# SEEDtk/kmers.anno

Hardware: AMD Instinct MI355X
Metric: kmer lookups/s + seqs annotated/s at 1/2/4/8 GPUs; achieved HBM GB/s vs roofline (higher is better)
Workload: dtype u64; 1 GPU; c5: 1M proteins per rank vs 10^8-entry multi-function signature table (HBM random access); proteins_per_gpu=1000000, windows_per_gpu=303576763, batch_windows=303576763, table_entries=100000000, functions=100000, k=8, min_hits=5, table_layout_m=6, table_minimizer_order=mod-sampling, table_placement=two-choice, parallelism=input-shard x1, table on this GPU

## Files before the change

kmers.anno_amd/csrc/kma_internal.h:

```cpp
#pragma once

#include <hip/hip_runtime.h>
#include <stdint.h>

#include "../../include/kmeranno.h"

namespace kma {

#ifndef KMA_BUCKET_SLOTS
#define KMA_BUCKET_SLOTS 8
#endif
constexpr int kSlotsPerBucket = KMA_BUCKET_SLOTS;
static_assert(kSlotsPerBucket == 8 || kSlotsPerBucket == 16, "64- or 128-byte buckets");
constexpr int kBucketBytes = kSlotsPerBucket * 8;
constexpr int kBucketHalves = kBucketBytes / 64;
constexpr int kSlotBits = kSlotsPerBucket == 16 ? 4 : 3;
#ifndef KMA_FILTER_BITS
#define KMA_FILTER_BITS 2
#endif
constexpr int kFilterBits = KMA_FILTER_BITS;
static_assert(kFilterBits >= 1 && kFilterBits <= 3, "one to three filter bits per slot");
constexpr uint32_t kFidBits = 24 - kFilterBits;
constexpr uint32_t kFidMask = (1u << kFidBits) - 1;
constexpr uint32_t kKeyHiMask = 0xFF000000u;
// ... 50 lines not shown
}
__host__ __device__ inline uint32_t mix32_lite(uint32_t h) {
  h ^= h >> 16;
  h *= 0x7FEB352Du;
  h ^= h >> 15;
  return h;
}
__host__ __device__ inline uint32_t parity32(uint32_t x) {
#ifdef __HIP_DEVICE_COMPILE__
  return (uint32_t)__popc(x) & 1u;
#else
  return (uint32_t)__builtin_popcount(x) & 1u;
#endif
}

__host__ __device__ inline uint32_t mmer_hash(uint32_t sub) {
#if KMA_HASH_LITE
  return sub * 0x9E3779B1u;
#else
  return mix32(sub * 0x9E3779B1u + 0x7F4A7C15u);
#endif
}
constexpr int kOrderMod = KMA_LAYOUT_MOD_SAMPLING;
constexpr int kMinimizerMask = 0x3F;
__host__ __device__ constexpr bool order_mod_valid(int k, int m) {
  return k == 8 && (m & kMinimizerMask) == 6;
}
__host__ __device__ inline uint32_t mod_sample(uint64_t key) {
  uint32_t best = 0xFFFFFFFFu;
  for (int i = 0; i < 8; ++i) {
    const uint32_t c = (uint32_t)(key >> (5 * (7 - i))) & 31u;
    const uint32_t g = (31u - c) << 5 | (uint32_t)(4 * i);
    best = best < g ? best : g;
  }
  const uint32_t lo = (uint32_t)key, hi = (uint32_t)(key >> 32);
#ifdef __HIP_DEVICE_COMPILE__
  const uint32_t sh = __builtin_amdgcn_ubfe(0x5A05A05Au, best, 4u);
  const uint32_t sub = __builtin_amdgcn_alignbit(hi, lo, sh) & 0x3FFFFFFFu;
#else
  const uint32_t sh = (0x5A05A05Au >> (best & 31u)) & 15u;
  const uint32_t sub = (uint32_t)(((uint64_t)hi << 32 | lo) >> sh) & 0x3FFFFFFFu;
#endif
  return mmer_hash(sub);
}
__host__ __device__ inline uint32_t minimizer_hash(uint64_t key, int k, int m) {
  if (m & kOrderMod) return mod_sample(key);
  const uint32_t mask = (uint32_t)((1ull << (5 * m)) - 1);
  uint32_t best = 0xFFFFFFFFu;
  for (int p = 0; p <= k - m; ++p) {
    const uint32_t h = mmer_hash((uint32_t)(key >> (5 * (k - m - p))) & mask);
    best = best < h ? best : h;
  }
  return best;
}

__host__ __device__ inline uint32_t home_from_hash(uint32_t h, uint64_t key, int m,
                                                   uint32_t n_buckets) {
  if (m != 0 && n_buckets >= 2) {
    const uint32_t pair = (uint32_t)(((uint64_t)h * (n_buckets >> 1)) >> 32);
#if KMA_HASH_LITE
    return 2u * pair + parity32((uint32_t)key);
#else
    return 2u * pair + (((uint32_t)key * 0x2C1B3C6Du) >> 31);
#endif
  }
  return (uint32_t)(((uint64_t)h * n_buckets) >> 32);
}
__host__ __device__ inline uint32_t home_from_min(uint32_t mn, uint64_t key, int m,
                                                  uint32_t n_buckets) {
#if KMA_HASH_LITE
  return home_from_hash(mix32_lite(mn ^ 0x85EBCA77u), key, m, n_buckets);
#else
  return home_from_hash(mix32(mn ^ 0x85EBCA77u), key, m, n_buckets);
#endif
}
__host__ __device__ inline uint32_t home_bucket(uint64_t key, int k, int m, uint32_t n_buckets) {
  if (m == 0)
    return home_from_hash(mix32((uint32_t)key ^ mix32((uint32_t)(key >> 32) + 0x9E3779B9u)),
                          key, m, n_buckets);
  return home_from_min(minimizer_hash(key, k, m), key, m, n_buckets);
}

#ifndef KMA_CHAIN_HASH
#define KMA_CHAIN_HASH 1
#endif
constexpr uint32_t kHashChainMin = 1024;
constexpr uint32_t kChainStepSearch = 4096;
__host__ __device__ inline bool chain_hashed(uint32_t n_buckets) {
  return KMA_CHAIN_HASH && n_buckets >= kHashChainMin;
}
__host__ __device__ inline uint32_t chain_bucket(uint32_t home, uint32_t i, uint32_t n_buckets) {
  if (chain_hashed(n_buckets)) {
    if (i == 0u) return home;
    const uint32_t r = (uint32_t)(((uint64_t)mix32(home * 0x9E3779B1u ^ i * 0x85EBCA77u) *
                                   (n_buckets - 1u)) >> 32);
    const uint32_t b = home + 1u + r;
    return b >= n_buckets ? b - n_buckets : b;
  }
  const uint64_t b = (uint64_t)home + i;
  return (uint32_t)(b >= n_buckets ? b - n_buckets : b);
}
__host__ __device__ inline uint32_t chain_step(uint32_t home, uint32_t b, uint32_t n_buckets) {
  if (chain_hashed(n_buckets)) {
    for (uint32_t i = 0; i < kChainStepSearch; ++i)
      if (chain_bucket(home, i, n_buckets) == b) return i;
    return kChainStepSearch;
  }
  return b >= home ? b - home : b + n_buckets - home;
}

__host__ __device__ inline uint32_t alt_bucket(uint64_t key, uint32_t home, uint32_t n_buckets) {
  const uint32_t h = mix32((uint32_t)key * 0x2C1B3C6Du ^ mix32_lite((uint32_t)(key >> 32) + 0x68E31DA5u));
  const uint32_t b = (uint32_t)(((uint64_t)h * (n_buckets - 1u)) >> 32);
  return b >= home ? b + 1u : b;
}
constexpr uint32_t kMaxKicks = 2000;
constexpr int kLayoutTwoChoice = KMA_LAYOUT_TWO_CHOICE;
constexpr int kLayoutMask = 0xFF;
constexpr double kMaxDisplacedTwoChoice = 0.40;

constexpr uint64_t kMinimizer6Buckets = kSlotsPerBucket == 16 ? (1ull << 24) : (1ull << 25);
constexpr uint64_t kMinimizer6BucketsWide = 1ull << 26;
int minimizer_len(int k, uint64_t n_buckets);
constexpr double kRetryDisplaced = 0.10;
constexpr double kMaxDisplaced = 0.15;
constexpr uint32_t kMaxChain = 32;

#ifndef KMA_BLOCK_PROTEINS
#define KMA_BLOCK_PROTEINS 8
#endif
#ifndef KMA_SET_POOL
#define KMA_SET_POOL 4096
#endif
#ifndef KMA_PROBE_WIN
#define KMA_PROBE_WIN (KMA_BUCKET_SLOTS == 16 ? 1 : 2)
#endif
constexpr int kProbeWin = KMA_PROBE_WIN;
constexpr int kBlockProteins = KMA_BLOCK_PROTEINS;
constexpr int kSetPool = KMA_SET_POOL;
#ifndef KMA_LANE_PERM
#define KMA_LANE_PERM 1
#endif
#ifndef KMA_CHAIN_Q
#define KMA_CHAIN_Q 192
#endif
constexpr int kChainQ = KMA_CHAIN_Q;
static_assert(kChainQ >= 64 * (kProbeWin + 1), "chain queue below two steps of windows");
constexpr uint32_t kGlobalSet = 0xFFFFFFFFu;
constexpr int kWavesPerBlock = 4;
#ifndef KMA_PROTEIN_OCC
#define KMA_PROTEIN_OCC 7
#endif
constexpr int kProteinOcc = KMA_PROTEIN_OCC;
#ifndef KMA_STAGE_RES
#define KMA_STAGE_RES 1024
#endif
constexpr int kStageRes = KMA_STAGE_RES;
constexpr int kStageGroups = kStageRes / 8 + 1;
constexpr int kStageEntries = (5 * kStageGroups + 15) / 16 * 4;
static_assert(kStageRes % (256 * kProbeWin) == 0, "a stage holds whole probe steps");
static_assert(4 * kStageEntries >= 5 * kStageRes / 8 + 8, "the last window reads two aligned words");
static_assert(kStageEntries < kSetPool / 2, "the stage leaves most of the pool to the sets");

struct ProteinArgs {
  const uint64_t* slots;
  uint32_t n_buckets;
  const uint8_t* lut;
  const uint8_t* residues;
  const uint64_t* offsets;
  uint32_t n_seq;
  uint32_t n_residues;
  int32_t k;
  int32_t mlen;
  int32_t min_hits;
  uint32_t flags;
  int32_t* out_fid;
  int32_t* out_count;
  uint8_t* out_status;
  uint32_t* tally;
  uint32_t n_fid;
  uint32_t* gset;
  uint32_t block_proteins;
  uint32_t defer_below;
  uint32_t n_groups;
  uint32_t packed;
  uint64_t stream_first;
  uint32_t two_choice;
};

struct ContigArgs {
  const uint64_t* slots;
  uint32_t n_buckets;
  const uint8_t* dna;
  const uint64_t* offsets;
  uint32_t n_contig;
  uint64_t total_bases;
  int32_t k;
  int32_t mlen;
  kma_hit* staging;
  uint32_t* block_counts;
  uint64_t* group_sum;
  uint32_t* emit_done;
  uint32_t n_groups;
  uint32_t groups_scanned;
  uint32_t* tally;
  uint32_t n_fid;
  kma_hit* out;
  uint64_t cap;
  uint64_t* n_hits;
  uint32_t* slot_count;
  int32_t strict_pass;
  uint32_t two_choice;
  uint8_t codon_codes[64];
};
#ifndef KMA_CONTIG_POS
#define KMA_CONTIG_POS 1
#endif
constexpr int kContigPos = KMA_CONTIG_POS;
#ifndef KMA_CONTIG_SEQ
#define KMA_CONTIG_SEQ 4
#endif
constexpr int kContigSeq = KMA_CONTIG_SEQ;
static_assert(kContigSeq == 1 || kContigPos == 1, "sequential slices take one position per lane");
constexpr int kContigTile = 256 * kContigPos * kContigSeq;
constexpr uint32_t kScanGroup = 256;
constexpr uint32_t kDirectGroups = 1024;

struct PropArgs {
  const kma_hit* hits;
  uint32_t n;
  const uint32_t* peg_len;
  uint32_t n_peg;
  int32_t k;
  double min_strength, max_fuzz, min_fuzz;
  uint32_t *keys, *skeys, *idx, *sidx;
  uint32_t *head, *list_no, *starts;
  uint32_t* scontig;
  int32_t* sleft;
  uint32_t *keep, *evidence, *out_pos;
  int32_t* best;
  uint64_t* stats;
  kma_proposal* out;
  uint64_t cap;
};
hipError_t launch_propose(PropArgs a, void* temp, size_t* temp_bytes, hipStream_t stream);

hipError_t launch_build_insert(uint64_t* slots, uint32_t* winner, uint32_t n_buckets, int k,
                               int m, const uint64_t* keys, uint64_t n, uint32_t* status,
                               hipStream_t stream);
hipError_t launch_build_finalize(uint64_t* slots, const uint32_t* winner, const uint32_t* fids,
                                 uint32_t n_buckets, int k, int m, uint32_t* stats,
                                 hipStream_t stream);
struct TwoChoiceScratch {
  uint32_t* home = nullptr;
  uint32_t* sorted_home = nullptr;
  uint32_t* sorted_idx = nullptr;
  uint8_t* away = nullptr;
  uint8_t* load = nullptr;
};
hipError_t launch_build_two_choice(uint64_t* slots, uint32_t n_buckets, int k, int m,
                                   const uint64_t* keys, const uint32_t* fids, uint64_t n,
                                   uint64_t* sorted_keys, uint32_t* rows, uint32_t* sorted_rows,
                                   const TwoChoiceScratch& x, void* temp, size_t* temp_bytes,
                                   uint32_t* status, hipStream_t stream);
hipError_t launch_annotate(const ProteinArgs& a, hipStream_t stream);
hipError_t launch_pack_residues(const uint8_t* residues, const uint64_t* offsets, uint64_t n,
                                const uint8_t* lut, uint8_t* out, hipStream_t stream);
__host__ __device__ constexpr uint64_t packed_bytes(uint64_t n) { return 40 * ((n + 63) / 64) + 16; }
hipError_t launch_contigs_emit(const ContigArgs& a, uint64_t n_blocks, hipStream_t stream);
hipError_t launch_contigs_probe(const ContigArgs& a, uint64_t n_blocks, hipStream_t stream);
hipError_t launch_peg_windows(const uint8_t* residues, const uint64_t* offsets, uint32_t n_peg,
                              int k, const uint8_t* lut, uint64_t* keys, uint32_t* pegs,
                              hipStream_t stream);
hipError_t launch_sort_pairs(void* temp, size_t* temp_bytes, const uint64_t* keys_in,
                             uint64_t* keys_out, const uint32_t* vals_in, uint32_t* vals_out,
                             uint64_t n, int key_bits, hipStream_t stream);
hipError_t launch_singleton_flags(const uint64_t* sorted_keys, uint64_t n, uint8_t* flags,
                                  hipStream_t stream);
constexpr uint32_t kBuildNeg = 0xFFFFFFu;
hipError_t launch_build_windows(const uint8_t* residues, const uint64_t* offsets, uint32_t n_seq,
                                const int32_t* roles, int k, int end_exclusive, const uint8_t* lut,
                                uint64_t* keys, uint32_t* tags, uint32_t* alpha_flag,
                                hipStream_t stream);
hipError_t launch_signature_flags(const uint64_t* keys, const uint32_t* tags, uint64_t n,
                                  uint8_t* flags, uint32_t* head_idx, uint32_t* run, void* temp,
                                  size_t* temp_bytes, hipStream_t stream);
hipError_t launch_select_flagged(void* temp, size_t* temp_bytes, const uint64_t* keys_in,
                                 const uint32_t* vals_in, const uint8_t* flags, uint64_t* keys_out,
                                 uint32_t* vals_out, uint64_t* n_out, uint64_t n,
                                 hipStream_t stream);

}
```

kmers.anno_amd/csrc/kma_kernels.hip:

```cpp
#include <cstring>
#include <rocprim/rocprim.hpp>

#include <algorithm>
#include <cstdio>
#include <cstdlib>

#include "../../include/kmeranno.h"
#include "kma_internal.h"
#include "kma_device.h"


namespace kma {
namespace {


template <bool Wide>
__global__ __launch_bounds__(256) void build_insert_kernel(uint64_t* slots, uint32_t* winner,
                                                           uint32_t n_buckets, int k, int m,
                                                           const uint64_t* __restrict__ keys,
                                                           uint64_t n, uint32_t* status) {
  constexpr int S = Wide ? kWideSlots : kSlotsPerBucket;
  for (uint64_t i = blockIdx.x * (uint64_t)blockDim.x + threadIdx.x; i < n;
       i += (uint64_t)gridDim.x * blockDim.x) {
    const uint64_t key = keys[i];
// ... 183 lines not shown
    while (e < n && hs[e] == h && e - i < 64) ++e;
    const uint32_t W = (uint32_t)(e - i);
    for (uint64_t j = i; j < e; ++j) away[ids[j]] = 0;
    if (W <= S) continue;
    uint64_t chosen = 0;
    uint32_t set = 0;
    for (uint32_t it = 0; it < W - S; ++it) {
      uint32_t best = 0, best_new = 64, best_mask = 0;
      for (uint32_t j = 0; j < W; ++j) {
        if (chosen >> j & 1ull) continue;
        const uint64_t key = skeys[ids[i + j]];
        const uint32_t mask = filter_need<S>((uint32_t)key);
        const bool alt_full = load && load[alt_bucket(key, h, n_buckets)] >= S;
        const uint32_t fresh = (uint32_t)__popc(mask & ~set) + (alt_full ? 32u : 0u);
        if (fresh < best_new) {
          best = j;
          best_new = fresh;
          best_mask = mask;
          if (fresh == 0) break;
        }
      }
      chosen |= 1ull << best;
      set |= best_mask;
      away[ids[i + best]] = 1;
    }
  }
}

__global__ __launch_bounds__(256) void build_two_choice_filter_kernel(uint64_t* slots,
                                                                      uint32_t n_buckets, int k,
                                                                      int m, uint32_t* stats) {
  constexpr int S = kSlotsPerBucket;
  const uint64_t n_slots = (uint64_t)n_buckets * S;
  uint32_t entries = 0, displaced = 0;
  for (uint64_t i = blockIdx.x * (uint64_t)blockDim.x + threadIdx.x; i < n_slots;
       i += (uint64_t)gridDim.x * blockDim.x) {
    const uint64_t v = __hip_atomic_load(slots + i, __ATOMIC_RELAXED, __HIP_MEMORY_SCOPE_AGENT);
    if ((uint32_t)v == 0u) continue;
    const uint64_t key = slot_key(v);
    const uint32_t b = (uint32_t)(i / S), h = home_bucket(key, k, m, n_buckets);
    entries++;
    if (b != h) {
      displaced++;
      for (int f = 0; f < kFilterBits; ++f) {
        const uint32_t pos = filter_pos<S>((uint32_t)key, f);
        uint32_t* meta = reinterpret_cast<uint32_t*>(slots + (uint64_t)h * S + pos / kFilterBits) + 1;
        const uint32_t bit = 1u << (kFidBits + pos % kFilterBits);
        if (!(__hip_atomic_load(meta, __ATOMIC_RELAXED, __HIP_MEMORY_SCOPE_AGENT) & bit))
          atomicOr(meta, bit);
      }
    }
  }
  entries = wave_sum(entries);
  displaced = wave_sum(displaced);
  if ((threadIdx.x & 63) == 0) {
    if (entries) atomicAdd(stats + 0, entries);
    atomicMax(stats + 1, displaced ? 2u : entries ? 1u : 0u);
    if (displaced) atomicAdd(stats + 2, displaced);
  }
}


#ifdef KMA_BLOCK_CLOCK
__device__ uint64_t g_block_clk[8 * 65536];
#define KMA_CLK_SET(i, v)                                          \
  do {                                                             \
    if (threadIdx.x == 0 && blockIdx.x < 65535)                    \
      g_block_clk[8 * blockIdx.x + (i)] = (v);                     \
  } while (0)
#define KMA_CLK(i) KMA_CLK_SET(i, wall_clock64())
#define KMA_CLK_HW()                                                \
  KMA_CLK_SET(6, (uint64_t)__builtin_amdgcn_s_getreg(20 | (15 << 11)) << 32 | \
                     (uint32_t)__builtin_amdgcn_s_getreg(4 | (31 << 11)))
#else
#define KMA_CLK_SET(i, v) ((void)0)
#define KMA_CLK(i) ((void)0)
#define KMA_CLK_HW() ((void)0)
#endif

#ifdef KMA_TUNE_COUNT
__device__ unsigned long long g_walk_stats[8];
#define KMA_COUNT(i, v)                                                                    \
  do {                                                                                     \
    const unsigned long long kma_v_ = (unsigned long long)(v);   \
    if ((threadIdx.x & 63) == 0)                                                           \
      __hip_atomic_fetch_add(&g_walk_stats[i], kma_v_, __ATOMIC_RELAXED,                   \
                             __HIP_MEMORY_SCOPE_AGENT);                                    \
  } while (0)
#else
#define KMA_COUNT(i, v) ((void)0)
#endif

template <int P>
struct ProteinSmem {
  __attribute__((aligned(16))) uint32_t pool[kSetPool];
  uint32_t chain_q[kWavesPerBlock][2 * kChainQ];
  uint32_t pbeg[P + 1];
  uint32_t pwin[P];
  uint32_t pset[P];
  uint32_t pcap[P];
  uint32_t pmin[P], pmax[P], pcnt[P];
  uint32_t plist[P];
  uint32_t skip;
  uint8_t lut[256];
};
static_assert(sizeof(ProteinSmem<kBlockProteins>) <= 163840 / kProteinOcc,
              "protein-path LDS must leave kProteinOcc blocks per CU");

__device__ __forceinline__ bool lds_set_insert(uint32_t* set, uint32_t cap, uint32_t key) {
  uint32_t i = set_slot(key, cap);
  for (;;) {
    const uint32_t o = atomicCAS(set + i, 0u, key);
    if (o == 0u) return true;
    if (o == key) return false;
    i = i + 1 == cap ? 0u : i + 1;
  }
}
__device__ __forceinline__ bool global_set_insert(uint32_t* set, uint32_t cap, uint32_t key) {
  uint32_t i = set_slot(key, cap);
  for (;;) {
    uint32_t o = 0u;
    __hip_atomic_compare_exchange_strong(set + i, &o, key, __ATOMIC_RELAXED, __ATOMIC_RELAXED,
                                         __HIP_MEMORY_SCOPE_AGENT);
    if (o == 0u) return true;
    if (o == key) return false;
    i = i + 1 == cap ? 0u : i + 1;
  }
}

template <int P>
__device__ __forceinline__ void record_hit(ProteinSmem<P>& sm, const ProteinArgs& a,
                                           uint64_t span_lo, bool multiset, uint32_t p,
                                           uint32_t fid, uint32_t sid) {
  atomicMin(&sm.pmin[p], fid);
  atomicMax(&sm.pmax[p], fid);
  bool fresh = true;
#ifdef KMA_TUNE_NO_SET
  fresh = false;
  if (false) {
#else
  if (!multiset) {
#endif
    const uint32_t base = sm.pset[p];
    if (base != kGlobalSet) {
      fresh = lds_set_insert(sm.pool + base, sm.pcap[p], sid + 1u);
    } else {
      a.gset[2 * (span_lo + sm.pbeg[p]) + atomicAdd(&sm.plist[p], 1u)] = sid + 1u;
      fresh = false;
    }
  }
  if (fresh) atomicAdd(&sm.pcnt[p], 1u);
}

template <int P>
__device__ __forceinline__ void dedupe_lists(ProteinSmem<P>& sm, const ProteinArgs& a,
                                             uint64_t span_lo) {
  const int t = threadIdx.x;
  for (int p = 0; p < P; ++p) {
    if (sm.pset[p] != kGlobalSet) continue;
    if (sm.pmin[p] != sm.pmax[p]) continue;
    const uint32_t h = sm.plist[p], b0 = sm.pbeg[p];
    if (h == 0) continue;
    const uint32_t* list = a.gset + 2 * (span_lo + b0);
    uint32_t fresh = 0;
    if (h < (uint32_t)kSetPool) {
      uint4* pool4 = reinterpret_cast<uint4*>(sm.pool);
      for (uint32_t i = t; i < (uint32_t)kSetPool / 4; i += 256) pool4[i] = make_uint4(0u, 0u, 0u, 0u);
      __syncthreads();
      for (uint32_t i = t; i < h; i += 256) fresh += lds_set_insert(sm.pool, kSetPool, list[i]);
    } else {
      const uint32_t L = sm.pbeg[p + 1] - b0;
      uint32_t* set = a.gset + 2 * (span_lo + b0) + L;
      for (uint32_t i = t; i < L; i += 256)
        __hip_atomic_store(set + i, 0u, __ATOMIC_RELAXED, __HIP_MEMORY_SCOPE_AGENT);
      __threadfence();
      __syncthreads();
      for (uint32_t i = t; i < h; i += 256) fresh += global_set_insert(set, L, list[i]);
    }
    fresh = wave_sum(fresh);
    if ((t & 63) == 0 && fresh) atomicAdd(&sm.pcnt[p], fresh);
    __syncthreads();
  }
}

template <int P>
__device__ __forceinline__ uint32_t dead_mask(const ProteinSmem<P>& sm) {
  uint32_t lane;
  asm volatile("v_mbcnt_lo_u32_b32 %0, -1, 0\n\tv_mbcnt_hi_u32_b32 %0, -1, %0" : "=v"(lane));
  const uint32_t i = lane < (uint32_t)P ? lane : 0u;
  const uint32_t mn = sm.pmin[i], mx = sm.pmax[i];
  return (uint32_t)__ballot(lane < (uint32_t)P && mx > mn);
}

template <int P>
__device__ __forceinline__ uint32_t protein_at(const uint32_t (&pb)[P + 1], uint32_t x) {
  uint32_t p = 0;
#pragma unroll
  for (int i = 1; i < P; ++i) p += x >= pb[i] ? 1u : 0u;
  return p;
}
template <int P>
__device__ __forceinline__ bool window_at(const uint32_t (&pe)[P], uint32_t x, uint32_t p) {
  uint32_t ended = 0;
#pragma unroll
  for (int i = 0; i < P; ++i) ended += x >= pe[i] ? 1u : 0u;
  return ended == p;
}

__device__ __forceinline__ uint32_t lane_window(int t) {
#if KMA_LANE_PERM
  return (uint32_t)((t >> 6) * 64 + 16 * (t & 3) + ((t & 63) >> 2));
#else
  return (uint32_t)t;
#endif
}

#ifndef KMA_XCD_GROUPS
#define KMA_XCD_GROUPS 1
#endif
__device__ __forceinline__ uint32_t xcd_group(uint32_t b, uint32_t n) {
#if KMA_XCD_GROUPS
  const uint32_t per = n >> 3;
  return b < 8u * per ? (b & 7u) * per + (b >> 3) : b;
#else
  (void)n;
  return b;
#endif
}

struct GroupHead {
  uint32_t p0, np;
  uint64_t beg_raw;
  uint64_t span_lo;
};
__device__ __forceinline__ void head_offsets(const ProteinArgs& a, uint32_t g, GroupHead& h) {
  const int lane = threadIdx.x & 63, wave = threadIdx.x >> 6;
  h.p0 = g * a.block_proteins;
  h.np = min(a.block_proteins, a.n_seq - h.p0);
  h.beg_raw = wave == 0 && lane <= (int)h.np ? a.offsets[h.p0 + lane] : 0u;
  h.span_lo = a.offsets[h.p0] - a.offsets[0];
}
template <bool Packed>
__device__ __forceinline__ const uint8_t* head_res(const ProteinArgs& a, const GroupHead& h,
                                                   uint64_t& pos0) {
  if (Packed) {
    pos0 = a.stream_first + h.span_lo;
    return a.residues;
  }
  const uint8_t* res0 = a.residues + a.offsets[0] + h.span_lo;
  pos0 = (uintptr_t)res0 & 7u;
  return res0 - pos0;
}
template <int U>
__device__ __forceinline__ void head_residues(const ProteinArgs& a, const GroupHead& h,
                                              uint32_t tw, WinWords (&ww)[U]) {
  uint64_t pos0;
  const uint8_t* res = head_res<true>(a, h, pos0);
  const uint64_t lim = a.n_residues - h.span_lo;
#pragma unroll
  for (int j = 0; j < U; ++j) {
    const uint32_t x = j * 256u + tw;
    ww[j] = window_words_packed(res, (x < lim ? x : 0u) + pos0);
  }
}

constexpr int kStagePerThread = (kStageGroups + 255) / 256;
static_assert(kStagePerThread <= kProbeWin, "a lane's stage words wait in its window registers");
__device__ __forceinline__ void stage_fetch(const uint8_t* __restrict__ res, uint32_t xc,
                                            uint32_t lim, WinWords (&ww)[kProbeWin]) {
  const uint64_t* words = reinterpret_cast<const uint64_t*>(res) + (xc >> 3);
#pragma unroll
  for (int i = 0; i < kStagePerThread; ++i) {
    const uint32_t g = threadIdx.x + 256u * i;
    const bool in = g < (uint32_t)kStageGroups && xc < lim && 8u * g < lim - xc;
    const uint64_t* src = in ? words + g : reinterpret_cast<const uint64_t*>(res);
    ww[i].lo = src[0];
    ww[i].hi = src[1];
  }
}
__device__ __forceinline__ void stage_store(uint8_t* stage, const uint8_t* lut, uint32_t sh,
                                            uint32_t xc, uint32_t lim,
                                            const WinWords (&ww)[kProbeWin]) {
#pragma unroll
  for (int i = 0; i < kStagePerThread; ++i) {
    const uint32_t g = threadIdx.x + 256u * i;
    if (g < (uint32_t)kStageGroups) {
      const bool in = xc < lim && 8u * g < lim - xc;
      store40(stage + 5u * g, in ? pack8(lut, funnel(ww[i].lo, ww[i].hi, sh)) : 0u);
    }
  }
}

template <int K, int M, int P, bool Packed>
__device__ __forceinline__ void annotate_block(const ProteinArgs& a, ProteinSmem<P>& sm,
                                               const GroupHead& h, WinWords (&ww)[kProbeWin],
                                               const int pass = -1) {
  constexpr uint32_t kPool = Packed ? kSetPool : kSetPool - kStageEntries;
  constexpr int U = kProbeWin;
  const int t = threadIdx.x, lane = t & 63, wave = t >> 6, part = t & 3;
  const bool multiset = (a.flags & KMA_F_MULTISET) != 0;
  const uint32_t tw = lane_window(t);
  const uint32_t p0 = h.p0, np = h.np;
  const uint64_t beg_raw = h.beg_raw, span_lo = h.span_lo;
  const uint64_t o0 = a.offsets[0];
  uint64_t pos0;
  const uint8_t* __restrict__ res = head_res<Packed>(a, h, pos0);
  if (wave == 0) {
    const uint64_t beg = lane <= (int)np ? beg_raw - o0 : 0u;
    const uint64_t end = __shfl_down(beg, 1, 64);
    const uint64_t lo = __shfl(beg, 0, 64), span_end = __shfl(beg, (int)np, 64);
    if (pass >= 0 && lane == 0) {
      const bool short_group = span_end - lo < (uint64_t)a.defer_below * 256u * kProbeWin;
      sm.skip = short_group != (pass == 1) ? 1u : 0u;
    }
    if (lane <= P) sm.pbeg[lane] = (uint32_t)((lane <= (int)np ? beg : span_end) - lo);
    if (lane < P) {
      uint32_t nw = 0;
      if (lane < (int)np) {
        const int64_t n = (int64_t)(end - beg) - K + ((a.flags & KMA_F_END_EXCLUSIVE) ? 0 : 1);
        nw = n > 0 ? (uint32_t)n : 0u;
      }
      sm.pwin[lane] = nw;
      sm.pcap[lane] = (nw == 0 || multiset) ? 0u : ((nw + (nw >> 1) + 4u) & ~3u);
      sm.pmin[lane] = 0xFFFFFFFFu;
      sm.pmax[lane] = 0u;
      sm.pcnt[lane] = 0u;
      sm.plist[lane] = 0u;
    }
    __builtin_amdgcn_wave_barrier();
    if (lane == 0) {
      uint32_t sum = 0;
      for (int p = 0; p < P; ++p) sum += sm.pcap[p];
      uint32_t top = 0;
      if (sum <= kPool) {
        for (int p = 0; p < P; ++p) {
          sm.pset[p] = top;
          top += sm.pcap[p];
        }
      } else {
        uint32_t done = 0;
        for (int it = 0; it < P; ++it) {
          int best = -1;
          for (int p = 0; p < P; ++p)
            if (!(done >> p & 1u) && (best < 0 || sm.pcap[p] > sm.pcap[best])) best = p;
          done |= 1u << best;
          const uint32_t cap = sm.pcap[best];
          const bool fits = top + cap <= kPool;
          sm.pset[best] = fits ? top : kGlobalSet;
          top += fits ? cap : 0u;
        }
      }
      sm.chain_q[0][0] = top;
    }
  }
  __syncthreads();
  if (pass >= 0 && sm.skip) return;
  uint8_t* stage = reinterpret_cast<uint8_t*>(sm.pool + kPool);
  const uint32_t stage_sh = (uint32_t)pos0 * 8u;
  if (!Packed) stage_store(stage, sm.lut, stage_sh, 0u, a.n_residues - (uint32_t)span_lo, ww);
  const uint32_t used = sm.chain_q[0][0];
  uint32_t pb[P + 1], pe[P];
#pragma unroll
  for (int i = 0; i <= P; ++i) pb[i] = __builtin_amdgcn_readfirstlane(sm.pbeg[i]);
#pragma unroll
  for (int i = 0; i < P; ++i) pe[i] = __builtin_amdgcn_readfirstlane(sm.pbeg[i] + sm.pwin[i]);
  const uint32_t span = pb[P];
  __syncthreads();
  uint4* pool4 = reinterpret_cast<uint4*>(sm.pool);
  KMA_CLK(1);
  for (uint32_t i = t; i < used / 4; i += 256) pool4[i] = make_uint4(0u, 0u, 0u, 0u);
  __syncthreads();

  const uint64_t* __restrict__ slots = a.slots;
  const uint32_t nb = a.n_buckets;
  const bool two_choice = a.two_choice != 0;
  uint32_t* cq = sm.chain_q[wave];
  uint32_t cn = 0;
  constexpr uint32_t stride = 256u * U;
  auto chain_flush = [&]() {
    __builtin_amdgcn_wave_barrier();
    KMA_COUNT(0, 1);
    KMA_COUNT(1, cn);
#ifdef KMA_TUNE_COUNT
    uint32_t wsum = 0, wmax = 0;
#endif
    const uint32_t dead_now = dead_mask<P>(sm);
    for (uint32_t e = lane; e < cn; e += 64) {
      const uint32_t w2 = cq[2 * e + 1];
      const uint64_t key = (uint64_t)(w2 & 0xFFu) << 32 | cq[2 * e];
      const uint32_t p = w2 >> 8;
      if (dead_now >> p & 1u) continue;
      uint32_t fid = 0, sid = 0;
#ifdef KMA_TUNE_COUNT
      uint32_t walked = 0;
      const bool hit = walk_chain(slots, nb, home_bucket(key, K, M, nb), key, fid, sid, two_choice,
                                  &walked);
#else
      const bool hit = walk_chain(slots, nb, home_bucket(key, K, M, nb), key, fid, sid, two_choice);
#endif
      if (hit) record_hit<P>(sm, a, span_lo, multiset, p, fid, sid);
#ifdef KMA_TUNE_COUNT
      {
        const uint32_t s1 = chain_bucket(home_bucket(key, K, M, nb), 1u, nb);
        const bool first = hit && sid / kSlotsPerBucket == s1;
        KMA_COUNT(4, __popcll(__ballot(hit)));
        KMA_COUNT(5, __popcll(__ballot(first)));
        wsum += walked;
        wmax = walked > wmax ? walked : wmax;
      }
#endif
    }
#ifdef KMA_TUNE_COUNT
    KMA_COUNT(6, wave_sum(wsum));
    KMA_COUNT(7, wave_max(wmax));
#endif
    __builtin_amdgcn_wave_barrier();
    cn = 0;
  };
  struct Prep {
    uint32_t klo[U], khi[U], need[U], bk[U];
  };
  auto prep = [&](uint32_t xs, Prep& o) {
#pragma unroll
    for (int j = 0; j < U; ++j) {
      const uint32_t x = xs + j * 256u + tw;
      const uint32_t p = protein_at<P>(pb, x);
      const uint64_t key = packed_key<K>(ww[j]);
      const bool ok = key != 0 && x < span && window_at<P>(pe, x, p);
      o.klo[j] = (uint32_t)key;
      o.khi[j] = (uint32_t)(key >> 32) << 24 | (ok ? 0u : 1u);
      o.need[j] = filter_need<kSlotsPerBucket>(o.klo[j]);
      o.bk[j] = p << kBucketBits | (ok ? home_bucket(key, K, M, nb) : 0u);
    }
  };
  auto gather = [&](const Prep& c, uint4 (&q)[U][4][kBucketHalves]) {
#pragma unroll
    for (int j = 0; j < U; ++j) {
      const uint32_t b0 = quad_bcast<0>(c.bk[j]), b1 = quad_bcast<1>(c.bk[j]);
      const uint32_t b2 = quad_bcast<2>(c.bk[j]), b3 = quad_bcast<3>(c.bk[j]);
      const uint32_t bb[4] = {b0, b1, b2, b3};
#pragma unroll
      for (int r = 0; r < 4; ++r) {
        const uint4* bp = reinterpret_cast<const uint4*>(slots) + part +
                          (uint64_t)(bb[r] & kBucketIdx) * kBucketQuads;
#pragma unroll
        for (int h = 0; h < kBucketHalves; ++h) q[j][r][h] = bp[4 * h];
      }
    }
  };
  auto load_residues = [&](uint32_t xs) {
#pragma unroll
    for (int j = 0; j < U; ++j) {
      const uint32_t x = xs + j * 256u + tw;
      if (Packed)
        ww[j] = window_words_packed(res, (x < span ? x : 0u) + pos0);
      else
        ww[j] = window_words_packed(stage, x % (uint32_t)kStageRes);
    }
  };
  auto settle = [&](uint32_t x0, const Prep& c, const uint4 (&q)[U][4][kBucketHalves]) {
    uint32_t word[U];
#pragma unroll
    for (int j = 0; j < U; ++j) {
      word[j] = 0;
      uint32_t raw[4];
      (void)raw;
#pragma unroll
      for (int r = 0; r < 4; ++r) {
        const uint32_t kl = r == 0 ? quad_bcast<0>(c.klo[j]) : r == 1 ? quad_bcast<1>(c.klo[j])
                          : r == 2 ? quad_bcast<2>(c.klo[j]) : quad_bcast<3>(c.klo[j]);
        const uint32_t kh = r == 0 ? quad_bcast<0>(c.khi[j]) : r == 1 ? quad_bcast<1>(c.khi[j])
                          : r == 2 ? quad_bcast<2>(c.khi[j]) : quad_bcast<3>(c.khi[j]);
        const uint32_t nd = r == 0 ? quad_bcast<0>(c.need[j]) : r == 1 ? quad_bcast<1>(c.need[j])
                          : r == 2 ? quad_bcast<2>(c.need[j]) : quad_bcast<3>(c.need[j]);
#if KMA_QUAD_XPOSE
        raw[r] = match_part_raw(q[j][r], kl, kh, nd, part);
#else
        const uint32_t v = match_part(q[j][r], kl, kh, nd, part);
        word[j] = part == r ? v : word[j];
#endif
      }
#if KMA_QUAD_XPOSE
      word[j] = quad_reduce_scatter(raw, part);
#endif
    }
#pragma unroll
    for (int j = 0; j < U; ++j) {
      const bool probed = (c.khi[j] & 1u) == 0u;
      const uint32_t w = probed ? word[j] : 0u;
#ifdef KMA_TUNE_COUNT
      KMA_COUNT(2, __popcll(__ballot(probed)));
      KMA_COUNT(3, __popcll(__ballot((w & kWordHit) != 0u)));
#endif
      if (w & kWordHit)
        record_hit<P>(sm, a, span_lo, multiset, c.bk[j] >> kBucketBits, w & kFidMask,
                      (c.bk[j] & kBucketIdx) * kSlotsPerBucket + ((w >> kSlotShift) & kSlotMask));
#ifdef KMA_TUNE_NO_WALK
      const bool pend = false;
#else
      const bool pend = probed && w == 0u;
#endif
      const uint64_t m = __ballot(pend);
      if (pend) {
        const uint32_t e = cn + popc_below(m);
        cq[2 * e] = c.klo[j];
        cq[2 * e + 1] = (c.khi[j] >> 24) | (c.bk[j] >> kBucketBits) << 8;
      }
      cn += (uint32_t)__popcll(m);
    }
    if (cn > (uint32_t)(kChainQ - 64 * U)) chain_flush();
  };
  if (!Packed) load_residues(0u);
  for (uint32_t x0 = 0; x0 < span; x0 += stride) {
    const uint32_t dead = dead_mask<P>(sm);
#pragma unroll
    for (int i = 0; i < P; ++i) pe[i] = dead >> i & 1u ? pb[i] : pe[i];
    Prep cur;
    prep(x0, cur);
    const uint32_t xn = x0 + stride;
    const bool restage = !Packed && xn % (uint32_t)kStageRes == 0u && xn < span;
    if (restage) stage_fetch(res, xn, span, ww);
    uint4 q[U][4][kBucketHalves];
    gather(cur, q);
    if (Packed) load_residues(xn);
    if (restage) {
      __syncthreads();
      stage_store(stage, sm.lut, stage_sh, xn, span, ww);
      __syncthreads();
    }
    settle(x0, cur, q);
    if (!Packed) load_residues(xn);
    if (x0 == 0) KMA_CLK(2);
  }
  KMA_CLK(3);
  KMA_CLK_SET(7, (span + stride - 1) / stride);
  if (cn) chain_flush();
  KMA_CLK(4);
  __syncthreads();
  if (!multiset) dedupe_lists<P>(sm, a, span_lo);
  if (t < (int)np) {
    const uint32_t mn = sm.pmin[t], mx = sm.pmax[t], cnt = sm.pcnt[t];
    int32_t fid_out = -1, cnt_out = 0;
    uint8_t st;
    if (mn == 0xFFFFFFFFu) {
      st = KMA_STATUS_NONE;
    } else if (mn != mx) {
      st = KMA_STATUS_AMBIGUOUS;
    } else {
      fid_out = (int32_t)mn;
      cnt_out = (int32_t)cnt;
      st = cnt >= (uint32_t)a.min_hits ? KMA_STATUS_CALLED : KMA_STATUS_BELOW_MIN;
      if (st == KMA_STATUS_CALLED && a.tally && mn < a.n_fid) atomicAdd(a.tally + mn, 1u);
    }
    a.out_fid[p0 + t] = fid_out;
    a.out_count[p0 + t] = cnt_out;
    a.out_status[p0 + t] = st;
  }
}

template <int K, int M, bool Packed>
constexpr int protein_occ() {
  return M == 0 ? 6 : kProteinOcc;
}
template <int K, int M, int P, bool Packed>
__global__ __launch_bounds__(256) __attribute__((amdgpu_waves_per_eu(protein_occ<K, M, Packed>(), 8))) void annotate_kernel(
    ProteinArgs a) {
  __shared__ ProteinSmem<P> sm;
  KMA_CLK(0);
  const int t = threadIdx.x;
  const uint8_t lut_b = Packed ? 0 : a.lut[t];
  const bool second = a.defer_below && blockIdx.x >= a.n_groups;
  GroupHead h;
  WinWords ww[kProbeWin];
  const uint32_t b = blockIdx.x - (second ? a.n_groups : 0u);
  head_offsets(a, a.defer_below ? b : xcd_group(b, a.n_groups), h);
  if (Packed) {
    head_residues<kProbeWin>(a, h, lane_window(t), ww);
  } else {
    uint64_t pos0;
    const uint8_t* res = head_res<false>(a, h, pos0);
    stage_fetch(res, 0u, a.n_residues - (uint32_t)h.span_lo, ww);
    sm.lut[t] = lut_b;
  }
  annotate_block<K, M, P, Packed>(a, sm, h, ww, a.defer_below ? (second ? 1 : 0) : -1);
  KMA_CLK(5);
  KMA_CLK_HW();
}

#ifdef KMA_TUNE_COUNT
}
}
extern "C" int kma_debug_walk_stats(uint64_t* out, int reset) {
  hipError_t e = hipMemcpyFromSymbol(out, HIP_SYMBOL(kma::g_walk_stats), 64, 0,
                                     hipMemcpyDeviceToHost);
  if (e == hipSuccess && reset) {
    const uint64_t z[8] = {};
    e = hipMemcpyToSymbol(HIP_SYMBOL(kma::g_walk_stats), z, 64, 0, hipMemcpyHostToDevice);
  }
  return (int)e;
}
namespace kma {
namespace {
#endif

#ifdef KMA_BLOCK_CLOCK
}
}
extern "C" int kma_debug_block_clock(uint64_t* out, uint64_t n) {
  return (int)hipMemcpyFromSymbol(out, HIP_SYMBOL(kma::g_block_clk), 8 * n, 0,
                                  hipMemcpyDeviceToHost);
}
namespace kma {
namespace {
#endif

__device__ __forceinline__ uint32_t contig_of(const uint64_t* __restrict__ off, uint32_t n,
                                              uint64_t g) {
  uint32_t lo = 0, hi = n;
  while (hi - lo > 1) {
    const uint32_t mid = (lo + hi) >> 1;
    if (off[mid] <= g) lo = mid; else hi = mid;
  }
  return lo;
}

__device__ __forceinline__ uint32_t base2(uint8_t c) {
  switch (c | 0x20) {
    case 't': case 'u': return 0u;
    case 'c': return 1u;
    case 'a': return 2u;
    case 'g': return 3u;
    default: return 4u;
  }
}


constexpr int kOffCache = 64;

__device__ __forceinline__ uint32_t contig_of_wave(const uint64_t* __restrict__ off, uint32_t n,
                                                   uint64_t g) {
  const uint32_t lane = threadIdx.x & 63;
  uint32_t lo = 0, span = n;
  while (span > 1) {
    const uint32_t step = (span + 63) / 64;
    const uint32_t c = lo + lane * step;
    const bool le = lane * step < span && off[c] <= g;
    const uint32_t k = (uint32_t)__popcll(__ballot(le)) - 1u;
    const uint32_t nlo = lo + k * step;
    span = min(step, lo + span - nlo);
    lo = nlo;
  }
  return lo;
}

#ifndef KMA_CONTIG_OCC
#define KMA_CONTIG_OCC (KMA_CONTIG_SEQ > 1 ? 7 : 8)
#endif
template <int K, int M>
__global__ __launch_bounds__(256) __attribute__((amdgpu_waves_per_eu(KMA_CONTIG_OCC, 8))) void contigs_probe_quad_kernel(
    ContigArgs a) {
  constexpr bool kWide = wide_k(K);
  constexpr int kS = kWide ? kWideSlots : kSlotsPerBucket;
  constexpr int kQ = kWide ? 4 : kBucketQuads;
  constexpr int kH = kWide ? 1 : kBucketHalves;
  constexpr int kSpan = kContigTile + 3 * K;
  __shared__ uint8_t bases[kSpan];
  __shared__ uint8_t aa_p[kSpan], aa_m[kSpan];
  __shared__ uint64_t offc[kOffCache + 1];
  __shared__ uint32_t crange[2];
  constexpr int CP = kContigPos * kContigSeq;
  __shared__ uint32_t wave_tot[kWavesPerBlock * CP];
  __shared__ uint8_t codon[64];
  const int t = threadIdx.x, lane = t & 63, wave = t >> 6, part = t & 3;
  const uint64_t base = ((const __attribute__((address_space(4))) uint64_t*)a.offsets)[0];
  const uint64_t end = base + a.total_bases;
  const uint64_t r0 = (uint64_t)blockIdx.x * kContigTile;
  const uint32_t nb = a.n_buckets;
  KMA_CLK(0);
  constexpr int kTileIters = (kSpan + 255) / 256;
  uint8_t tb[kTileIters];
#pragma unroll
  for (int j = 0; j < kTileIters; ++j) {
    const int i = t + 256 * j;
    const uint64_t g = base + r0 + i;
    tb[j] = i < kSpan && g < end ? a.dna[g] : (uint8_t)'N';
  }
  if (wave == 3) codon[lane] = a.codon_codes[lane];
  if (a.n_contig < (uint32_t)kOffCache) {
    if (wave == 0) {
      const uint32_t n = a.n_contig;
      const uint64_t last = r0 + kContigTile < a.total_bases ? r0 + kContigTile : a.total_bases;
      const uint64_t v = a.offsets[min((uint32_t)lane, n)];
      const uint32_t lo = (uint32_t)__popcll(__ballot((uint32_t)lane < n && v <= base + r0)) - 1u;
      const uint32_t hi =
          (uint32_t)__popcll(__ballot((uint32_t)lane < n && v <= base + last - 1)) - 1u;
      offc[lane] = __shfl(v, (int)min(lo + (uint32_t)lane, n), 64);
      const uint64_t vn = __shfl(v, (int)n, 64);
      if (lane == 0) {
        offc[kOffCache] = vn;
        crange[0] = lo;
        crange[1] = hi;
      }
    }
  } else if (wave < 2) {
    const uint64_t last = r0 + kContigTile < a.total_bases ? r0 + kContigTile : a.total_bases;
    const uint32_t c = contig_of_wave(a.offsets, a.n_contig, base + (wave ? last - 1 : r0));
    if (lane == 0) crange[wave] = c;
    if (wave == 0) {
      offc[lane] = a.offsets[min(c + lane, a.n_contig)];
      if (lane == 0) offc[kOffCache] = a.offsets[min(c + kOffCache, a.n_contig)];
    }
  }
#pragma unroll
  for (int j = 0; j < kTileIters; ++j) {
    const int i = t + 256 * j;
    if (i < kSpan) bases[i] = (uint8_t)(base + r0 + i < end ? base2(tb[j]) : 4u);
  }
  __syncthreads();
  KMA_CLK(1);
  const uint32_t c_lo = crange[0], nc = crange[1] - c_lo + 1;
  for (int i = t; i < kSpan - 2; i += blockDim.x) {
    const uint32_t b0 = bases[i], b1 = bases[i + 1], b2 = bases[i + 2];
    if ((b0 | b1 | b2) & 4u) {
      aa_p[i] = aa_m[i] = 0;
    } else {
      aa_p[i] = codon[b0 * 16 + b1 * 4 + b2];
      aa_m[i] = codon[(b2 ^ 2u) * 16 + (b1 ^ 2u) * 4 + (b0 ^ 2u)];
    }
  }
  __syncthreads();
  KMA_CLK(2);

  constexpr int CL = kContigPos;
#if KMA_LANE_PERM
// ... 646 lines not shown
```

Measured before the change: 128.4 billion kmer lookups/s.

## Split each block's residue span into contiguous per-wave chunks instead of interleaved steps

Changes the window-to-lane mapping so each wave/unroll slot walks its own contiguous chunk of the block's residue span, with the step count computed per group from the offsets. The LDS staging buffer is restructured into per-slot regions holding two steps each, and several indices are made wave-uniform (scalar) via readfirstlane and asm constraints. The intent is to cut per-window address arithmetic, make staging refills rarer, and improve locality. The risks are load imbalance across slots at the tail of the span and more complex stage indexing.

```diff
diff --git a/kmers.anno_amd/csrc/kma_internal.h b/kmers.anno_amd/csrc/kma_internal.h
--- a/kmers.anno_amd/csrc/kma_internal.h
+++ b/kmers.anno_amd/csrc/kma_internal.h
@@ -226,14 +226,15 @@
 #define KMA_PROTEIN_OCC 7
 #endif
 constexpr int kProteinOcc = KMA_PROTEIN_OCC;
-#ifndef KMA_STAGE_RES
-#define KMA_STAGE_RES 1024
-#endif
-constexpr int kStageRes = KMA_STAGE_RES;
-constexpr int kStageGroups = kStageRes / 8 + 1;
+constexpr int kStepSlots = kWavesPerBlock * kProbeWin;
+constexpr int kStageSteps = 2;
+constexpr int kRegionGroups = 64 * kStageSteps / 8 + 1;
+constexpr int kRegionRes = 8 * kRegionGroups;
+constexpr int kStageGroups = kStepSlots * kRegionGroups;
 constexpr int kStageEntries = (5 * kStageGroups + 15) / 16 * 4;
-static_assert(kStageRes % (256 * kProbeWin) == 0, "a stage holds whole probe steps");
-static_assert(4 * kStageEntries >= 5 * kStageRes / 8 + 8, "the last window reads two aligned words");
+static_assert(4 * kStageEntries >=
+                  5 * (kRegionRes * (kStepSlots - 1) + 64 * kStageSteps - 1) / 8 / 8 * 8 + 16,
+              "the last window reads two aligned words");
 static_assert(kStageEntries < kSetPool / 2, "the stage leaves most of the pool to the sets");
 
 struct ProteinArgs {
diff --git a/kmers.anno_amd/csrc/kma_kernels.hip b/kmers.anno_amd/csrc/kma_kernels.hip
--- a/kmers.anno_amd/csrc/kma_kernels.hip
+++ b/kmers.anno_amd/csrc/kma_kernels.hip
@@ -359,10 +359,15 @@
   if (fresh) atomicAdd(&sm.pcnt[p], 1u);
 }
 
+__device__ __forceinline__ uint32_t lane_id() {
+  uint32_t lane;
+  asm volatile("v_mbcnt_lo_u32_b32 %0, -1, 0\n\tv_mbcnt_hi_u32_b32 %0, -1, %0" : "=v"(lane));
+  return lane;
+}
+
 template <int P>
 __device__ __forceinline__ void dedupe_lists(ProteinSmem<P>& sm, const ProteinArgs& a,
-                                             uint64_t span_lo) {
-  const int t = threadIdx.x;
+                                             uint64_t span_lo, const int t) {
   for (int p = 0; p < P; ++p) {
     if (sm.pset[p] != kGlobalSet) continue;
     if (sm.pmin[p] != sm.pmax[p]) continue;
@@ -392,8 +397,7 @@
 
 template <int P>
 __device__ __forceinline__ uint32_t dead_mask(const ProteinSmem<P>& sm) {
-  uint32_t lane;
-  asm volatile("v_mbcnt_lo_u32_b32 %0, -1, 0\n\tv_mbcnt_hi_u32_b32 %0, -1, %0" : "=v"(lane));
+  const uint32_t lane = lane_id();
   const uint32_t i = lane < (uint32_t)P ? lane : 0u;
   const uint32_t mn = sm.pmin[i], mx = sm.pmax[i];
   return (uint32_t)__ballot(lane < (uint32_t)P && mx > mn);
@@ -414,12 +418,19 @@
   return ended == p;
 }
 
-__device__ __forceinline__ uint32_t lane_window(int t) {
+__device__ __forceinline__ uint32_t chunk_window(int t) {
 #if KMA_LANE_PERM
-  return (uint32_t)((t >> 6) * 64 + 16 * (t & 3) + ((t & 63) >> 2));
+  return (uint32_t)(16 * (t & 3) + ((t & 63) >> 2));
 #else
-  return (uint32_t)t;
-#endif
+  return (uint32_t)(t & 63);
+#endif
+}
+__device__ __forceinline__ uint32_t chunk_pos(uint32_t r, uint32_t T, uint32_t s) {
+  return 64u * (r * T + s);
+}
+__device__ __forceinline__ uint32_t scalar_whole(uint32_t v) {
+  asm volatile("" : "+s"(v));
+  return v;
 }
 
 #ifndef KMA_XCD_GROUPS
@@ -437,6 +448,7 @@
 
 struct GroupHead {
   uint32_t p0, np;
+  uint32_t steps;
   uint64_t beg_raw;
   uint64_t span_lo;
 };
@@ -445,7 +457,9 @@
   h.p0 = g * a.block_proteins;
   h.np = min(a.block_proteins, a.n_seq - h.p0);
   h.beg_raw = wave == 0 && lane <= (int)h.np ? a.offsets[h.p0 + lane] : 0u;
-  h.span_lo = a.offsets[h.p0] - a.offsets[0];
+  const uint64_t lo = a.offsets[h.p0], hi = a.offsets[h.p0 + h.np];
+  h.span_lo = lo - a.offsets[0];
+  h.steps = (uint32_t)((hi - lo + 256u * kProbeWin - 1u) / (256u * kProbeWin));
 }
 template <bool Packed>
 __device__ __forceinline__ const uint8_t* head_res(const ProteinArgs& a, const GroupHead& h,
@@ -460,39 +474,44 @@
 }
 template <int U>
 __device__ __forceinline__ void head_residues(const ProteinArgs& a, const GroupHead& h,
-                                              uint32_t tw, WinWords (&ww)[U]) {
+                                              uint32_t wave, uint32_t cw, WinWords (&ww)[U]) {
   uint64_t pos0;
   const uint8_t* res = head_res<true>(a, h, pos0);
   const uint64_t lim = a.n_residues - h.span_lo;
 #pragma unroll
   for (int j = 0; j < U; ++j) {
-    const uint32_t x = j * 256u + tw;
+    const uint32_t x = chunk_pos(kWavesPerBlock * j + wave, h.steps, 0u) + cw;
     ww[j] = window_words_packed(res, (x < lim ? x : 0u) + pos0);
   }
 }
 
 constexpr int kStagePerThread = (kStageGroups + 255) / 256;
 static_assert(kStagePerThread <= kProbeWin, "a lane's stage words wait in its window registers");
-__device__ __forceinline__ void stage_fetch(const uint8_t* __restrict__ res, uint32_t xc,
-                                            uint32_t lim, WinWords (&ww)[kProbeWin]) {
-  const uint64_t* words = reinterpret_cast<const uint64_t*>(res) + (xc >> 3);
+__device__ __forceinline__ uint32_t stage_group_pos(uint32_t g, uint32_t T, uint32_t s) {
+  const uint32_t r = g / (uint32_t)kRegionGroups;
+  return chunk_pos(r, T, s) + 8u * (g - r * (uint32_t)kRegionGroups);
+}
+__device__ __forceinline__ void stage_fetch(const uint8_t* __restrict__ res, uint32_t T,
+                                            uint32_t s, uint32_t lim, WinWords (&ww)[kProbeWin]) {
+  const uint64_t* words = reinterpret_cast<const uint64_t*>(res);
 #pragma unroll
   for (int i = 0; i < kStagePerThread; ++i) {
     const uint32_t g = threadIdx.x + 256u * i;
-    const bool in = g < (uint32_t)kStageGroups && xc < lim && 8u * g < lim - xc;
-    const uint64_t* src = in ? words + g : reinterpret_cast<const uint64_t*>(res);
+    const uint32_t x = stage_group_pos(g, T, s);
+    const bool in = g < (uint32_t)kStageGroups && x < lim;
+    const uint64_t* src = words + (in ? x >> 3 : 0u);
     ww[i].lo = src[0];
     ww[i].hi = src[1];
   }
 }
 __device__ __forceinline__ void stage_store(uint8_t* stage, const uint8_t* lut, uint32_t sh,
-                                            uint32_t xc, uint32_t lim,
+                                            uint32_t T, uint32_t s, uint32_t lim,
                                             const WinWords (&ww)[kProbeWin]) {
 #pragma unroll
   for (int i = 0; i < kStagePerThread; ++i) {
     const uint32_t g = threadIdx.x + 256u * i;
     if (g < (uint32_t)kStageGroups) {
-      const bool in = xc < lim && 8u * g < lim - xc;
+      const bool in = stage_group_pos(g, T, s) < lim;
       store40(stage + 5u * g, in ? pack8(lut, funnel(ww[i].lo, ww[i].hi, sh)) : 0u);
     }
   }
@@ -506,7 +525,10 @@
   constexpr int U = kProbeWin;
   const int t = threadIdx.x, lane = t & 63, wave = t >> 6, part = t & 3;
   const bool multiset = (a.flags & KMA_F_MULTISET) != 0;
-  const uint32_t tw = lane_window(t);
+  const uint32_t T = h.steps;
+  const uint32_t ws = (uint32_t)__builtin_amdgcn_readfirstlane(wave);
+  const uint32_t wv = Packed ? 0u : ws;
+  const uint32_t cw = chunk_window(t) + (Packed ? chunk_pos((uint32_t)wave, T, 0u) : 0u);
   const uint32_t p0 = h.p0, np = h.np;
   const uint64_t beg_raw = h.beg_raw, span_lo = h.span_lo;
   const uint64_t o0 = a.offsets[0];
@@ -564,7 +586,7 @@
   if (pass >= 0 && sm.skip) return;
   uint8_t* stage = reinterpret_cast<uint8_t*>(sm.pool + kPool);
   const uint32_t stage_sh = (uint32_t)pos0 * 8u;
-  if (!Packed) stage_store(stage, sm.lut, stage_sh, 0u, a.n_residues - (uint32_t)span_lo, ww);
+  if (!Packed) stage_store(stage, sm.lut, stage_sh, T, 0u, a.n_residues - (uint32_t)span_lo, ww);
   const uint32_t used = sm.chain_q[0][0];
   uint32_t pb[P + 1], pe[P];
 #pragma unroll
@@ -581,9 +603,8 @@
   const uint64_t* __restrict__ slots = a.slots;
   const uint32_t nb = a.n_buckets;
   const bool two_choice = a.two_choice != 0;
-  uint32_t* cq = sm.chain_q[wave];
+  uint32_t* cq = sm.chain_q[ws];
   uint32_t cn = 0;
-  constexpr uint32_t stride = 256u * U;
   auto chain_flush = [&]() {
     __builtin_amdgcn_wave_barrier();
     KMA_COUNT(0, 1);
@@ -592,7 +613,7 @@
     uint32_t wsum = 0, wmax = 0;
 #endif
     const uint32_t dead_now = dead_mask<P>(sm);
-    for (uint32_t e = lane; e < cn; e += 64) {
+    for (uint32_t e = lane_id(); e < cn; e += 64) {
       const uint32_t w2 = cq[2 * e + 1];
       const uint64_t key = (uint64_t)(w2 & 0xFFu) << 32 | cq[2 * e];
       const uint32_t p = w2 >> 8;
@@ -627,10 +648,11 @@
   struct Prep {
     uint32_t klo[U], khi[U], need[U], bk[U];
   };
-  auto prep = [&](uint32_t xs, Prep& o) {
+  auto prep = [&](uint32_t s, Prep& o) {
 #pragma unroll
     for (int j = 0; j < U; ++j) {
-      const uint32_t x = xs + j * 256u + tw;
+      const uint32_t xc = chunk_pos(kWavesPerBlock * j + wv, T, s);
+      const uint32_t x = (Packed ? xc : scalar_whole(xc)) + cw;
       const uint32_t p = protein_at<P>(pb, x);
       const uint64_t key = packed_key<K>(ww[j]);
       const bool ok = key != 0 && x < span && window_at<P>(pe, x, p);
@@ -655,17 +677,20 @@
       }
     }
   };
-  auto load_residues = [&](uint32_t xs) {
+  auto load_residues = [&](uint32_t s) {
 #pragma unroll
     for (int j = 0; j < U; ++j) {
-      const uint32_t x = xs + j * 256u + tw;
-      if (Packed)
+      const uint32_t r = kWavesPerBlock * j + wv;
+      if (Packed) {
+        const uint32_t x = chunk_pos(r, T, s) + cw;
         ww[j] = window_words_packed(res, (x < span ? x : 0u) + pos0);
-      else
-        ww[j] = window_words_packed(stage, x % (uint32_t)kStageRes);
+      } else {
+        const uint32_t at = (uint32_t)kRegionRes * r + 64u * (s % (uint32_t)kStageSteps);
+        ww[j] = window_words_packed(stage, scalar_whole(at) + cw);
+      }
     }
   };
-  auto settle = [&](uint32_t x0, const Prep& c, const uint4 (&q)[U][4][kBucketHalves]) {
+  auto settle = [&](const Prep& c, const uint4 (&q)[U][4][kBucketHalves]) {
     uint32_t word[U];
 #pragma unroll
     for (int j = 0; j < U; ++j) {
@@ -718,34 +743,36 @@
     if (cn > (uint32_t)(kChainQ - 64 * U)) chain_flush();
   };
   if (!Packed) load_residues(0u);
-  for (uint32_t x0 = 0; x0 < span; x0 += stride) {
+  for (uint32_t s = 0; s < T; ++s) {
     const uint32_t dead = dead_mask<P>(sm);
 #pragma unroll
     for (int i = 0; i < P; ++i) pe[i] = dead >> i & 1u ? pb[i] : pe[i];
     Prep cur;
-    prep(x0, cur);
-    const uint32_t xn = x0 + stride;
-    const bool restage = !Packed && xn % (uint32_t)kStageRes == 0u && xn < span;
-    if (restage) stage_fetch(res, xn, span, ww);
+    prep(s, cur);
+    const uint32_t sn = s + 1u;
+    const bool restage = !Packed && sn % (uint32_t)kStageSteps == 0u && sn < T;
+    if (restage) stage_fetch(res, T, sn, span, ww);
     uint4 q[U][4][kBucketHalves];
     gather(cur, q);
-    if (Packed) load_residues(xn);
+    if (Packed) load_residues(sn);
     if (restage) {
       __syncthreads();
-      stage_store(stage, sm.lut, stage_sh, xn, span, ww);
+      stage_store(stage, sm.lut, stage_sh, T, sn, span, ww);
       __syncthreads();
     }
-    settle(x0, cur, q);
-    if (!Packed) load_residues(xn);
-    if (x0 == 0) KMA_CLK(2);
+    settle(cur, q);
+    if (!Packed) load_residues(sn);
+    if (s == 0) KMA_CLK(2);
   }
   KMA_CLK(3);
-  KMA_CLK_SET(7, (span + stride - 1) / stride);
+  KMA_CLK_SET(7, T);
   if (cn) chain_flush();
   KMA_CLK(4);
   __syncthreads();
-  if (!multiset) dedupe_lists<P>(sm, a, span_lo);
-  if (t < (int)np) {
+  const int te = (int)(64u * ws + lane_id());
+  if (!multiset) dedupe_lists<P>(sm, a, span_lo, te);
+  if (te < (int)np) {
+    const int t = te;
     const uint32_t mn = sm.pmin[t], mx = sm.pmax[t], cnt = sm.pcnt[t];
     int32_t fid_out = -1, cnt_out = 0;
     uint8_t st;
@@ -782,11 +809,11 @@
   const uint32_t b = blockIdx.x - (second ? a.n_groups : 0u);
   head_offsets(a, a.defer_below ? b : xcd_group(b, a.n_groups), h);
   if (Packed) {
-    head_residues<kProbeWin>(a, h, lane_window(t), ww);
+    head_residues<kProbeWin>(a, h, (uint32_t)t >> 6, chunk_window(t), ww);
   } else {
     uint64_t pos0;
     const uint8_t* res = head_res<false>(a, h, pos0);
-    stage_fetch(res, 0u, a.n_residues - (uint32_t)h.span_lo, ww);
+    stage_fetch(res, h.steps, 0u, a.n_residues - (uint32_t)h.span_lo, ww);
     sm.lut[t] = lut_b;
   }
   annotate_block<K, M, P, Packed>(a, sm, h, ww, a.defer_below ? (second ? 1 : 0) : -1);
```

Result: faster. 137.7 billion kmer lookups/s (median of 6 runs) (+7.3%).
